# pepborrell/cool-chic

Measured on AMD Instinct MI355X. Metric: decoded Mpixel/s (Synth+ARM+upsample) @1280x720, all GPUs, higher is better.
Workload: dtype f32; 1 GPU; 1280x720 YUV420 8-bit frames, hop/c3x decoder (arm 16x2, syn 48-1/3-1/3-3r/3-3r, 7 latent grids), float forward ARM+rate -> upsampling -> synthesis -> 420 post; parallelism=image-parallel x1, kernels=ARM | upsampling pyramid | fused last-upsampling+synthesis+post (one stream)

## Files before the change

### cool-chic_amd/ccmi/__init__.py

```python

from __future__ import annotations

import ctypes as C
import os
from pathlib import Path

PKG_ROOT = Path(__file__).resolve().parents[1]
LIB_PATH = Path(os.environ.get("CCMI_LIB", PKG_ROOT / "lib" / "libccmi.so"))

MAX_GRIDS = 8
MAX_SYN_LAYERS = 16

OK, ERR_ARG, ERR_HIP, ERR_UNSUPPORTED, ERR_BITSTREAM, ERR_IO = range(6)

EXPORTED = [
    "ccmi_last_error", "ccmi_version", "ccmi_device_count",
    "ccmi_arm_forward_f32", "ccmi_arm_context_f32", "ccmi_arm_mlp_f32", "ccmi_ups_workspace_bytes", "ccmi_ups_forward_f32",
    "ccmi_syn_workspace_bytes", "ccmi_syn_forward_f32", "ccmi_post_f32", "ccmi_decode_forward_f32",
    "ccmi_fused_run_plan",
    "ccmi_decode_file", "ccmi_decode_batch", "ccmi_decode_output_size", "ccmi_decode_last_timing",
    "ccmi_decode_last_arm_flags", "ccmi_decode_latents", "ccmi_decode_batch_workspace_bytes", "ccmi_decode_batch_plan", "ccmi_decode_batch_ws", "ccmi_decode_weights_i32",
    "ccmi_decode_batch_dev_plan", "ccmi_decode_batch_dev", "ccmi_decode_batch_dev_roi_plan", "ccmi_decode_batch_dev_roi",
    "ccmi_latents_plan", "ccmi_latents_decode", "ccmi_latents_free", "ccmi_latents_count", "ccmi_latents_values",
    "ccmi_latents_render_plan", "ccmi_latents_render",
    "ccmi_latents_compact_plan", "ccmi_latents_compact_measure", "ccmi_latents_compact", "ccmi_latents_concat",
    "ccmi_latents_stream_info",
    "ccmi_latents_file_head", "ccmi_latents_export_plan", "ccmi_latents_export", "ccmi_latents_import_plan",
    "ccmi_latents_import",
    "ccmi_decode_batch_dev_fmt_plan", "ccmi_decode_batch_dev_fmt", "ccmi_latents_render_fmt_plan", "ccmi_latents_render_fmt",
    "ccmi_decode_batch_dev_rs_plan", "ccmi_decode_batch_dev_rs", "ccmi_latents_render_rs_plan", "ccmi_latents_render_rs",
    "ccmi_decode_last_tail_groups",
    "ccmi_decode_batch_dev_warp_plan", "ccmi_decode_batch_dev_warp", "ccmi_latents_render_warp_plan", "ccmi_latents_render_warp",
    "ccmi_decode_batch_dev_col_plan", "ccmi_decode_batch_dev_col", "ccmi_latents_render_col_plan", "ccmi_latents_render_col",
    "ccmi_ups_workspace_bytes_i32", "ccmi_ups_forward_i32", "ccmi_syn_workspace_bytes_i32", "ccmi_syn_forward_i32",
    "ccmi_cool_parse", "ccmi_code_wb", "ccmi_decode_wb", "ccmi_code_latent_layer", "ccmi_arm_forward_i32",
    "ccmi_encode_frame", "ccmi_row_reduce_f32", "ccmi_train_param_count", "ccmi_train_workspace_bytes", "ccmi_train_step",
    "ccmi_quantize_f32",
]


class CcmiUnavailable(RuntimeError):
    pass


class CcmiError(RuntimeError):
    def __init__(self, code: int, msg: str):
        super().__init__(f"ccmi error {code}: {msg}")
        self.code = code


class ArmArgs(C.Structure):
    _fields_ = [
        ("latent", C.c_void_p), ("latent_stride", C.c_int64), ("n_grids", C.c_int),
        ("h", C.c_int * MAX_GRIDS), ("w", C.c_int * MAX_GRIDS), ("gain", C.c_float),
        ("quantize", C.c_int), ("dim_arm", C.c_int), ("n_hidden", C.c_int),
        ("params", C.c_void_p), ("param_stride", C.c_int64),
        ("mu", C.c_void_p), ("scale", C.c_void_p), ("log_scale", C.c_void_p), ("rate", C.c_void_p),
        ("out_stride", C.c_int64), ("batch", C.c_int),
    ]


class UpsArgs(C.Structure):
    _fields_ = [
        ("latent", C.c_void_p), ("latent_stride", C.c_int64), ("n_grids", C.c_int),
        ("h", C.c_int * MAX_GRIDS), ("w", C.c_int * MAX_GRIDS), ("gain", C.c_float),
        ("quantize", C.c_int), ("ups_k", C.c_int), ("n_ups", C.c_int), ("pre_k", C.c_int),
        ("n_pre", C.c_int), ("params", C.c_void_p), ("param_stride", C.c_int64),
        ("out", C.c_void_p), ("out_stride", C.c_int64), ("workspace", C.c_void_p),
        ("workspace_bytes", C.c_size_t), ("batch", C.c_int),
    ]


class SynLayer(C.Structure):
    _fields_ = [("n_out", C.c_int), ("ks", C.c_int), ("residual", C.c_int), ("relu", C.c_int)]


class SynArgs(C.Structure):
    _fields_ = [
        ("in_", C.c_void_p), ("in_stride", C.c_int64), ("c_in", C.c_int), ("h", C.c_int), ("w", C.c_int),
        ("n_layers", C.c_int), ("layers", SynLayer * MAX_SYN_LAYERS), ("params", C.c_void_p),
        ("param_stride", C.c_int64), ("out", C.c_void_p), ("out_stride", C.c_int64),
        ("workspace", C.c_void_p), ("workspace_bytes", C.c_size_t), ("batch", C.c_int),
    ]


class PostArgs(C.Structure):
    _fields_ = [
        ("in_", C.c_void_p), ("in_stride", C.c_int64), ("h", C.c_int), ("w", C.c_int),
        ("bitdepth", C.c_int), ("yuv420", C.c_int), ("out", C.c_void_p), ("out_stride", C.c_int64),
        ("batch", C.c_int),
    ]


class DecodeArgs(C.Structure):
    _fields_ = [
        ("ups", UpsArgs), ("syn", SynArgs), ("bitdepth", C.c_int), ("yuv420", C.c_int),
        ("out", C.c_void_p), ("out_stride", C.c_int64), ("stages", C.c_int), ("head", C.c_int),
    ]


HEAD_DEFAULT, HEAD_VALU, HEAD_MFMA, HEAD_GENERIC = 0, 1, 2, 3


_lib = None


def lib() -> C.CDLL:
    global _lib
    if _lib is not None:
        return _lib
    try:
        import torch
    except ImportError:
        pass
    if not LIB_PATH.exists():
        raise CcmiUnavailable(f"{LIB_PATH} not built: run `make -C cool-chic_amd` (or __graft_entry__.build())")
    L = C.CDLL(str(LIB_PATH))
    L.ccmi_last_error.restype = C.c_char_p
    L.ccmi_version.restype = C.c_int
    L.ccmi_device_count.restype = C.c_int
    for name, st in (("ccmi_arm_forward_f32", ArmArgs), ("ccmi_ups_forward_f32", UpsArgs),
                     ("ccmi_syn_forward_f32", SynArgs), ("ccmi_post_f32", PostArgs),
                     ("ccmi_decode_forward_f32", DecodeArgs)):
        f = getattr(L, name)
        f.argtypes = [C.POINTER(st), C.c_void_p]
        f.restype = C.c_int
    L.ccmi_arm_context_f32.argtypes = [C.c_void_p, C.c_int, C.c_int, C.c_int, C.c_int, C.c_void_p, C.c_void_p]
    L.ccmi_arm_context_f32.restype = C.c_int
    L.ccmi_arm_mlp_f32.argtypes = [C.c_void_p, C.c_int64, C.c_int, C.c_int, C.c_void_p, C.c_void_p, C.c_void_p,
                                   C.c_void_p, C.c_void_p]
    L.ccmi_arm_mlp_f32.restype = C.c_int
    L.ccmi_ups_workspace_bytes.argtypes = [C.c_int, C.POINTER(C.c_int), C.POINTER(C.c_int), C.c_int]
    L.ccmi_ups_workspace_bytes.restype = C.c_size_t
    L.ccmi_syn_workspace_bytes.argtypes = [C.POINTER(SynArgs)]
    L.ccmi_syn_workspace_bytes.restype = C.c_size_t
    L.ccmi_decode_file.argtypes = [C.c_char_p, C.c_char_p, C.c_int, C.c_int, C.c_int, C.c_int]
    L.ccmi_decode_file.restype = C.c_int
    L.ccmi_decode_batch.argtypes = [C.POINTER(C.c_void_p), C.POINTER(C.c_size_t), C.c_int,
                                    C.POINTER(C.c_void_p), C.POINTER(C.c_size_t), C.POINTER(C.c_size_t),
                                    C.c_int, C.c_int, C.c_int, C.c_void_p]
    L.ccmi_decode_batch.restype = C.c_int
    L.ccmi_decode_output_size.argtypes = [C.c_void_p, C.c_size_t, C.c_int, C.c_int, C.c_int,
                                          C.POINTER(C.c_size_t)]
    L.ccmi_decode_output_size.restype = C.c_int
    L.ccmi_decode_last_timing.argtypes = [C.POINTER(C.c_float)]
    L.ccmi_decode_last_timing.restype = C.c_int
    if hasattr(L, "ccmi_fused_run_plan"):
        L.ccmi_fused_run_plan.argtypes = [C.c_int, C.c_int, C.c_int, C.POINTER(C.c_int), C.POINTER(C.c_int), C.c_int,
                                          C.POINTER(C.c_int)]
        L.ccmi_fused_run_plan.restype = C.c_int
    if hasattr(L, "ccmi_decode_last_arm_flags"):
        L.ccmi_decode_last_arm_flags.argtypes = [C.POINTER(C.c_uint32), C.c_int, C.POINTER(C.c_int)]
        L.ccmi_decode_last_arm_flags.restype = C.c_int
    _lib = L
    return L


def check(rc: int) -> None:
    if rc != OK:
        raise CcmiError(rc, lib().ccmi_last_error().decode(errors="replace"))


def last_error() -> str:
    return lib().ccmi_last_error().decode(errors="replace")


def __getattr__(name):
    if name == "LatentStore":
        from .decode import LatentStore
        return LatentStore
    raise AttributeError(f"module 'ccmi' has no attribute {name!r}")


def stream_handle(device=None) -> int:
    import torch
    return torch.cuda.current_stream(device).cuda_stream


def ptr(t) -> int:
# ... 12 lines not shown
```

### cool-chic_amd/ccmi/forward.py

```python

from __future__ import annotations

import ctypes
from typing import Sequence

import torch

from . import (ArmArgs, DecodeArgs, MAX_GRIDS, MAX_SYN_LAYERS, PostArgs, SynArgs, SynLayer, UpsArgs, check, lib, ptr,
               require_cuda, stream_handle)


def _grid_arrays(sizes: Sequence[tuple[int, int]]):
    if not 1 <= len(sizes) <= MAX_GRIDS:
        raise ValueError(f"1..{MAX_GRIDS} latent grids supported, got {len(sizes)}")
    h = (ctypes.c_int * MAX_GRIDS)()
    w = (ctypes.c_int * MAX_GRIDS)()
    for i, (hh, ww) in enumerate(sizes):
        h[i], w[i] = int(hh), int(ww)
    return h, w


def n_latents(sizes) -> int:
    return sum(int(h) * int(w) for h, w in sizes)


def arm_param_count(dim_arm: int, n_hidden: int) -> int:
    return n_hidden * (dim_arm * dim_arm + dim_arm) + 2 * dim_arm + 2


def pack_arm(layers: Sequence[tuple[torch.Tensor, torch.Tensor]]) -> torch.Tensor:
    return torch.cat([t.reshape(-1).float() for wb in layers for t in wb])


def pack_ups(ups: Sequence[torch.Tensor], pre: Sequence[torch.Tensor]) -> torch.Tensor:
    return torch.cat([k.reshape(-1).float() for k in list(ups) + list(pre)])


def pack_syn(layers: Sequence[tuple[torch.Tensor, torch.Tensor]]) -> torch.Tensor:
    return torch.cat([t.reshape(-1).float() for wb in layers for t in wb])


def _as_batch(params: torch.Tensor, B: int):
    if params.dim() == 1:
        return params.unsqueeze(0), 0
    if params.shape[0] != B:
        raise ValueError(f"params: expected {B} parameter rows, got {params.shape[0]}")
    return params, params.shape[1]


def arm_forward(latent: torch.Tensor, sizes, params: torch.Tensor, dim_arm: int, n_hidden: int,
                gain: float = 16.0, quantize: bool = True, want=("mu", "scale", "log_scale", "rate")) -> dict:
    squeeze = latent.dim() == 1
    latent = latent.unsqueeze(0) if squeeze else latent
    B, N = latent.shape
    params, pstride = _as_batch(params, B)
    require_cuda(latent, params)
    if N != n_latents(sizes):
        raise ValueError(f"latent has {N} values, grids hold {n_latents(sizes)}")
    if params.shape[1] < arm_param_count(dim_arm, n_hidden):
        raise ValueError("arm params: expected [B, >=%d]" % arm_param_count(dim_arm, n_hidden))
    latent = latent.float().contiguous()
    params = params.float().contiguous()
    outs = {k: torch.empty(B, N, device=latent.device, dtype=torch.float32) for k in want}
    h, w = _grid_arrays(sizes)
    a = ArmArgs(latent=ptr(latent), latent_stride=N, n_grids=len(sizes), h=h, w=w, gain=float(gain),
                quantize=int(bool(quantize)), dim_arm=dim_arm, n_hidden=n_hidden, params=ptr(params),
                param_stride=pstride, mu=ptr(outs.get("mu")), scale=ptr(outs.get("scale")),
                log_scale=ptr(outs.get("log_scale")), rate=ptr(outs.get("rate")), out_stride=N, batch=B)
    check(lib().ccmi_arm_forward_f32(a, stream_handle(latent.device)))
    if squeeze:
        outs = {k: v[0] for k, v in outs.items()}
    return outs


def ups_forward(latent: torch.Tensor, sizes, params: torch.Tensor, ups_k: int, n_ups: int, pre_k: int, n_pre: int,
                gain: float = 16.0, quantize: bool = True) -> torch.Tensor:
    squeeze = latent.dim() == 1
    latent = latent.unsqueeze(0) if squeeze else latent
    B, N = latent.shape
    params, pstride = _as_batch(params, B)
    require_cuda(latent, params)
    if N != n_latents(sizes):
        raise ValueError(f"latent has {N} values, grids hold {n_latents(sizes)}")
    if params.shape[1] < n_ups * ups_k + n_pre * pre_k:
        raise ValueError("ups params: wrong shape")
    latent = latent.float().contiguous()
    params = params.float().contiguous()
    L = len(sizes)
    H, W = sizes[0]
    out = torch.empty(B, L, H, W, device=latent.device, dtype=torch.float32)
    h, w = _grid_arrays(sizes)
    nws = lib().ccmi_ups_workspace_bytes(L, h, w, B)
    ws = torch.empty(max(nws, 4), device=latent.device, dtype=torch.uint8)
    a = UpsArgs(latent=ptr(latent), latent_stride=N, n_grids=L, h=h, w=w, gain=float(gain),
                quantize=int(bool(quantize)), ups_k=ups_k, n_ups=n_ups, pre_k=pre_k, n_pre=n_pre,
                params=ptr(params), param_stride=pstride, out=ptr(out), out_stride=L * H * W,
                workspace=ptr(ws), workspace_bytes=nws, batch=B)
    check(lib().ccmi_ups_forward_f32(a, stream_handle(latent.device)))
    return out[0] if squeeze else out


def _syn_args(x, layers, params, out, B, C, H, W, pstride=None):
    if len(layers) > MAX_SYN_LAYERS:
        raise ValueError("too many synthesis layers")
    arr = (SynLayer * MAX_SYN_LAYERS)()
    for i, (n_out, ks, res, relu) in enumerate(layers):
        arr[i] = SynLayer(int(n_out), int(ks), int(bool(res)), int(bool(relu)))
    return SynArgs(in_=ptr(x), in_stride=C * H * W, c_in=C, h=H, w=W, n_layers=len(layers), layers=arr,
                   params=ptr(params), param_stride=params.shape[1] if pstride is None else pstride, out=ptr(out),
                   out_stride=out.shape[1] * H * W, workspace=None, workspace_bytes=0, batch=B)


def syn_param_count(c_in: int, layers) -> int:
    n, c = 0, c_in
    for n_out, ks, _, _ in layers:
        n += n_out * c * ks * ks + n_out
        c = n_out
    return n


def syn_forward(x: torch.Tensor, layers, params: torch.Tensor) -> torch.Tensor:
    squeeze = x.dim() == 3
# ... 124 lines not shown
```

### cool-chic_amd/csrc/ccmi_api.cpp

```cpp
#include <stdarg.h>
#include <stdio.h>

#include <mutex>

#include "ccmi_internal.h"

static thread_local char g_err[512] = "";

int ccmi_set_error(int code, const char *fmt, ...)
{
    va_list ap;
    va_start(ap, fmt);
    vsnprintf(g_err, sizeof g_err, fmt, ap);
    va_end(ap);
    return code;
}

static std::mutex g_pool_mu;
static std::vector<StreamSet *> g_pool;

StreamSet *ccmi_streamset_acquire(int nst, int nev, bool timing)
{
    int dev = 0;
    if (hipGetDevice(&dev) != hipSuccess) {
        ccmi_set_error(CCMI_ERR_HIP, "stream pool: hipGetDevice failed");
        return nullptr;
    }
    {
        std::lock_guard<std::mutex> lk(g_pool_mu);
        for (size_t i = 0; i < g_pool.size(); ++i) {
            StreamSet *s = g_pool[i];
            if (s->device == dev && s->timing == timing && (int)s->st.size() >= nst && (int)s->ev.size() >= nev) {
                g_pool.erase(g_pool.begin() + (long)i);
                return s;
            }
        }
    }
    StreamSet *s = new StreamSet;
    s->device = dev;
    s->timing = timing;
    s->st.assign(nst, nullptr);
    s->ev.assign(nev, nullptr);
    bool ok = true;
    for (auto &x : s->st) ok = ok && hipStreamCreateWithFlags(&x, hipStreamNonBlocking) == hipSuccess;
    for (auto &x : s->ev) ok = ok && (timing ? hipEventCreate(&x) : hipEventCreateWithFlags(&x, hipEventDisableTiming)) == hipSuccess;
    if (!ok) {
        ccmi_set_error(CCMI_ERR_HIP, "stream pool: stream / event creation failed");
        for (auto x : s->st)
            if (x) (void)hipStreamDestroy(x);
        for (auto x : s->ev)
            if (x) (void)hipEventDestroy(x);
        delete s;
        return nullptr;
    }
    return s;
}

void ccmi_streamset_release(StreamSet *set)
{
    std::lock_guard<std::mutex> lk(g_pool_mu);
    g_pool.push_back(set);
}

extern "C" const char *ccmi_last_error(void) { return g_err; }

extern "C" int ccmi_version(void) { return 101; }

extern "C" int ccmi_device_count(void)
{
    int n = 0;
    if (hipGetDeviceCount(&n) != hipSuccess) return 0;
    return n;
}

static int check_grids(int n, const int *h, const int *w, const char *who)
{
    if (n < 1 || n > CCMI_MAX_GRIDS) return ccmi_set_error(CCMI_ERR_ARG, "%s: n_grids must be in [1, %d]", who, CCMI_MAX_GRIDS);
    for (int l = 0; l < n; ++l)
        if (h[l] < 1 || w[l] < 1) return ccmi_set_error(CCMI_ERR_ARG, "%s: grid %d has size %dx%d", who, l, h[l], w[l]);
    return CCMI_OK;
}

extern "C" int ccmi_arm_forward_f32(const ccmi_arm_args *a, void *stream)
{
    if (!a || !a->latent || !a->params) return ccmi_set_error(CCMI_ERR_ARG, "arm: null argument");
    if (int rc = check_grids(a->n_grids, a->h, a->w, "arm")) return rc;
    if (a->batch < 1) return ccmi_set_error(CCMI_ERR_ARG, "arm: batch must be >= 1");
    if (a->n_hidden < 0 || a->n_hidden > 4) return ccmi_set_error(CCMI_ERR_UNSUPPORTED, "arm: n_hidden must be in [0, 4]");
    const int64_t need = (int64_t)a->n_hidden * (a->dim_arm * a->dim_arm + a->dim_arm) + 2 * a->dim_arm + 2;
    if (a->param_stride != 0 && a->param_stride < need) return ccmi_set_error(CCMI_ERR_ARG, "arm: param_stride < %lld", (long long)need);
    if (!a->rate && !a->mu && !a->scale && !a->log_scale) return ccmi_set_error(CCMI_ERR_ARG, "arm: no output requested");
    return ccmi_launch_arm_f32(a, static_cast<hipStream_t>(stream));
}

extern "C" int ccmi_ups_forward_f32(const ccmi_ups_args *a, void *stream)
{
    if (!a || !a->latent || !a->params || !a->out) return ccmi_set_error(CCMI_ERR_ARG, "ups: null argument");
    if (int rc = check_grids(a->n_grids, a->h, a->w, "ups")) return rc;
    if (a->batch < 1) return ccmi_set_error(CCMI_ERR_ARG, "ups: batch must be >= 1");
    return ccmi_launch_ups_f32(a, static_cast<hipStream_t>(stream));
}

extern "C" int ccmi_syn_forward_f32(const ccmi_syn_args *a, void *stream)
{
    if (!a || !a->in || !a->params || !a->out) return ccmi_set_error(CCMI_ERR_ARG, "syn: null argument");
    if (a->h < 1 || a->w < 1 || a->c_in < 1 || a->batch < 1) return ccmi_set_error(CCMI_ERR_ARG, "syn: bad shape");
    return ccmi_launch_syn_f32(a, static_cast<hipStream_t>(stream));
}

extern "C" int ccmi_post_f32(const ccmi_post_args *a, void *stream)
{
    if (!a || !a->in || !a->out) return ccmi_set_error(CCMI_ERR_ARG, "post: null argument");
    if (a->h < 1 || a->w < 1 || a->batch < 1) return ccmi_set_error(CCMI_ERR_ARG, "post: bad shape");
    return ccmi_launch_post_f32(a, static_cast<hipStream_t>(stream));
}
```

### cool-chic_amd/csrc/ccmi_internal.h

```cpp
#pragma once

#include <hip/hip_runtime.h>
#include <stdint.h>

#include <vector>

#include "../../include/ccmi.h"

#define CCMI_MAX_GRIDS 8

struct GridGeom {
    int n;
    int h[CCMI_MAX_GRIDS];
    int w[CCMI_MAX_GRIDS];
    int off[CCMI_MAX_GRIDS];
    int total;
};

int ccmi_set_error(int code, const char *fmt, ...);

#define CCMI_HIP_CHECK(expr)                                                                \
    do {                                                                                    \
        hipError_t _e = (expr);                                                             \
        if (_e != hipSuccess)                                                               \
            return ccmi_set_error(CCMI_ERR_HIP, "%s failed: %s", #expr, hipGetErrorString(_e)); \
    } while (0)

static inline int ccmi_div_up(int a, int b) { return (a + b - 1) / b; }

int ccmi_launch_arm_f32(const ccmi_arm_args *a, hipStream_t s);
int ccmi_launch_ups_f32(const ccmi_ups_args *a, hipStream_t s);
int ccmi_launch_syn_f32(const ccmi_syn_args *a, hipStream_t s);
int ccmi_launch_post_f32(const ccmi_post_args *a, hipStream_t s);

struct StreamSet {
    int device = -1;
    bool timing = false;
    std::vector<hipStream_t> st;
    std::vector<hipEvent_t> ev;
};
StreamSet *ccmi_streamset_acquire(int nst, int nev, bool timing);
void ccmi_streamset_release(StreamSet *set);
struct StreamSetLease {
    StreamSet *set = nullptr;
    StreamSetLease() = default;
    StreamSetLease(const StreamSetLease &) = delete;
    StreamSetLease &operator=(const StreamSetLease &) = delete;
    ~StreamSetLease()
    {
        if (set) ccmi_streamset_release(set);
    }
};
```

### cool-chic_amd/csrc/fwd_arm.hip

```cpp
#include <stdlib.h>

#include <algorithm>

#include "fwd_common.h"

using ccmi_fwd::cfloat_ptr;
using ccmi_fwd::f2;

namespace {

constexpr int kThreads = 256;
constexpr int kTX = 64;
constexpr int kRowsPerPass = kThreads / kTX;
#ifndef CCMI_ARM_NL
#define CCMI_ARM_NL 2
#endif
constexpr int kNL = CCMI_ARM_NL;
constexpr int kNP = kNL / 2;
constexpr int kTY = kRowsPerPass * kNL;
constexpr int kHalo = 4;
constexpr int kLW = kTX + 2 * kHalo;
constexpr int kLH = kTY + kHalo;


struct ArmGeom {
    int n;
    int h[CCMI_MAX_GRIDS], w[CCMI_MAX_GRIDS], off[CCMI_MAX_GRIDS];
    int tiles_x[CCMI_MAX_GRIDS];
    int tile_start[CCMI_MAX_GRIDS + 1];
};

template <int D>
__device__ __forceinline__ void ctx_offset(int i, int &dy, int &dx)
{
    constexpr signed char k8[8] = {13, 22, 30, 31, 32, 37, 38, 39};
    constexpr signed char k16[16] = {13, 14, 20, 21, 22, 23, 24, 28, 29, 30, 31, 32, 33, 37, 38, 39};
    constexpr signed char k24[24] = {4, 11, 12, 13, 14, 15, 19, 20, 21, 22, 23, 24, 25, 28, 29, 30, 31, 32, 33, 34,
                                     36, 37, 38, 39};
    constexpr signed char k32[32] = {2, 3, 4, 5, 10, 11, 12, 13, 14, 15, 16, 19, 20, 21, 22, 23, 24, 25, 26, 27,
                                     28, 29, 30, 31, 32, 33, 34, 35, 36, 37, 38, 39};
    int k = D == 8 ? k8[i] : D == 16 ? k16[i] : D == 24 ? k24[i] : k32[i];
    dy = k / 9 - 4;
    dx = k % 9 - 4;
}

__device__ __forceinline__ float laplace_cdf(float x, float mu, float inv_scale)
{
    float s = x - mu;
    float sg = s > 0.f ? 1.f : (s < 0.f ? -1.f : 0.f);
    return 0.5f - 0.5f * sg * (__expf(-fabsf(s) * inv_scale) - 1.f);
}

template <int D, int NH = -1>
__global__ __launch_bounds__(kThreads) void arm_fwd_kernel(
    const float *__restrict__ lat, int64_t lat_stride, ArmGeom g, float gain, int quantize, int nh,
    const float *__restrict__ params, int64_t pstride, float *__restrict__ o_mu, float *__restrict__ o_scale,
    float *__restrict__ o_log_scale, float *__restrict__ o_rate, int64_t ostride)
{
    __shared__ float tile[kLH][kLW];

    const int wt = ccmi_fwd::xcd_order(blockIdx.x, gridDim.x);
    const int ntl = g.tile_start[g.n];
    const int b = wt / ntl;
    const int t = wt - b * ntl;
    int l = 0;
#pragma unroll
    for (int k = 1; k < CCMI_MAX_GRIDS; ++k)
        if (k < g.n && t >= g.tile_start[k]) l = k;
    const int lt = t - g.tile_start[l];
    const int H = g.h[l], W = g.w[l];
    const int y0 = (lt / g.tiles_x[l]) * kTY;
    const int x0 = (lt % g.tiles_x[l]) * kTX;
    const float *src = lat + (int64_t)b * lat_stride + g.off[l];

    {
        constexpr int NU = (kLH * kLW + kThreads - 1) / kThreads;
        float lv[NU];
#pragma unroll
        for (int u = 0; u < NU; ++u) {
            const int i = threadIdx.x + u * kThreads;
            const int r = i / kLW, c = i - r * kLW;
            const int y = y0 - kHalo + r, x = x0 - kHalo + c;
            lv[u] = (i < kLH * kLW && y >= 0 && y < H && x >= 0 && x < W) ? src[y * W + x] : 0.f;
        }
#pragma unroll
        for (int u = 0; u < NU; ++u) {
            const int i = threadIdx.x + u * kThreads;
            if (i < kLH * kLW) tile[i / kLW][i % kLW] = quantize ? rintf(gain * lv[u]) : lv[u];
        }
    }
    __syncthreads();

    const cfloat_ptr p = (cfloat_ptr)(size_t)(params + (int64_t)b * pstride);
    const int cx = threadIdx.x % kTX;
    const int cy0 = threadIdx.x / kTX;

    static_assert(kNL % 2 == 0, "packed pair layout");
    f2 a[kNP][D];
#pragma unroll
    for (int i = 0; i < D; ++i) {
        int dy, dx;
        ctx_offset<D>(i, dy, dx);
#pragma unroll
        for (int q = 0; q < kNP; ++q)
            a[q][i] = f2{tile[cy0 + 2 * q * kRowsPerPass + kHalo + dy][cx + kHalo + dx],
                         tile[cy0 + (2 * q + 1) * kRowsPerPass + kHalo + dy][cx + kHalo + dx]};
    }

    if constexpr (NH >= 0) nh = NH;
#pragma unroll
    for (int layer = 0; layer < nh; ++layer) {
        const cfloat_ptr Wl = p + layer * (D * D + D);
        const cfloat_ptr bl = Wl + D * D;
        f2 o[kNP][D];
#pragma unroll
        for (int j = 0; j < D; ++j) {
            f2 acc[kNP];
#pragma unroll
            for (int q = 0; q < kNP; ++q) acc[q] = a[q][j] + f2(bl[j]);
#pragma unroll
            for (int i = 0; i < D; ++i) {
                const f2 wji = f2(Wl[j * D + i]);
#pragma unroll
                for (int q = 0; q < kNP; ++q) acc[q] = __builtin_elementwise_fma(wji, a[q][i], acc[q]);
            }
#pragma unroll
            for (int q = 0; q < kNP; ++q) o[q][j] = __builtin_elementwise_max(acc[q], f2(0.f));
        }
#pragma unroll
        for (int q = 0; q < kNP; ++q)
#pragma unroll
            for (int j = 0; j < D; ++j) a[q][j] = o[q][j];
    }

    const cfloat_ptr Wo = p + nh * (D * D + D);
    f2 m[kNP], ls[kNP];
#pragma unroll
    for (int q = 0; q < kNP; ++q) {
        m[q] = f2(Wo[2 * D]);
        ls[q] = f2(Wo[2 * D + 1]);
    }
#pragma unroll
    for (int i = 0; i < D; ++i) {
        const f2 w0 = f2(Wo[i]), w1 = f2(Wo[D + i]);
#pragma unroll
        for (int q = 0; q < kNP; ++q) {
            m[q] = __builtin_elementwise_fma(w0, a[q][i], m[q]);
            ls[q] = __builtin_elementwise_fma(w1, a[q][i], ls[q]);
        }
    }
#pragma unroll
    for (int n = 0; n < kNL; ++n) {
        const int y = y0 + cy0 + n * kRowsPerPass, x = x0 + cx;
        const float mn = (n & 1) ? m[n >> 1].y : m[n >> 1].x, lsn = (n & 1) ? ls[n >> 1].y : ls[n >> 1].x;
        if (y < H && x < W) {
            const float sc = __expf(fminf(fmaxf(lsn - 4.f, -4.6f), 5.0f));
            const float q = tile[cy0 + n * kRowsPerPass + kHalo][cx + kHalo];
            const int64_t idx = (int64_t)b * ostride + g.off[l] + y * W + x;
            if (o_mu) o_mu[idx] = mn;
            if (o_scale) o_scale[idx] = sc;
            if (o_log_scale) o_log_scale[idx] = lsn;
            if (o_rate) {
                const float is = __builtin_amdgcn_rcpf(sc);
                const float pr = fmaxf(laplace_cdf(q + 0.5f, mn, is) - laplace_cdf(q - 0.5f, mn, is), 1.52587890625e-05f);
                o_rate[idx] = -__log2f(pr);
            }
        }
    }
}

template <int D>
__global__ __launch_bounds__(kThreads) void arm_context_kernel(const float *__restrict__ grid, int H, int W,
                                                               float *__restrict__ out)
{
    const int b = blockIdx.y;
    const int64_t p = (int64_t)blockIdx.x * kThreads + threadIdx.x;
    if (p >= (int64_t)H * W) return;
    const int y = (int)(p / W), x = (int)(p - (int64_t)y * W);
    const float *g = grid + (int64_t)b * H * W;
    float *o = out + ((int64_t)b * H * W + p) * D;
#pragma unroll
    for (int i = 0; i < D; ++i) {
        int dy, dx;
        ctx_offset<D>(i, dy, dx);
        const int yy = y + dy, xx = x + dx;
        o[i] = (yy >= 0 && xx >= 0 && xx < W) ? g[yy * W + xx] : 0.f;
    }
}

template <int D>
__global__ __launch_bounds__(kThreads) void arm_mlp_kernel(const float *__restrict__ ctx, int64_t M, int nh,
                                                           const float *__restrict__ p, float *__restrict__ o_mu,
                                                           float *__restrict__ o_scale, float *__restrict__ o_ls)
{
    const int64_t r = (int64_t)blockIdx.x * kThreads + threadIdx.x;
    if (r >= M) return;
    float a[D];
#pragma unroll
    for (int i = 0; i < D; ++i) a[i] = ctx[r * D + i];
    for (int layer = 0; layer < nh; ++layer) {
        const float *Wl = p + layer * (D * D + D);
        float o[D];
#pragma unroll
        for (int j = 0; j < D; ++j) {
            float acc = 0.f;
#pragma unroll
            for (int i = 0; i < D; ++i) acc = fmaf(Wl[j * D + i], a[i], acc);
            o[j] = fmaxf((acc + Wl[D * D + j]) + a[j], 0.f);
        }
#pragma unroll
        for (int j = 0; j < D; ++j) a[j] = o[j];
    }
    const float *Wo = p + nh * (D * D + D);
    float m = 0.f, ls = 0.f;
#pragma unroll
    for (int i = 0; i < D; ++i) {
        m = fmaf(Wo[i], a[i], m);
        ls = fmaf(Wo[D + i], a[i], ls);
    }
    m += Wo[2 * D];
    ls += Wo[2 * D + 1];
    if (o_mu) o_mu[r] = m;
    if (o_ls) o_ls[r] = ls;
    if (o_scale) o_scale[r] = expf(fminf(fmaxf(ls - 4.f, -4.6f), 5.0f));
}

}

extern "C" int ccmi_arm_context_f32(const float *grid, int batch, int h, int w, int dim_arm, float *out, void *stream)
{
    if (!grid || !out || batch < 1 || h < 1 || w < 1) return ccmi_set_error(CCMI_ERR_ARG, "arm_context: bad argument");
    dim3 g((unsigned)(((int64_t)h * w + kThreads - 1) / kThreads), batch);
    hipStream_t s = static_cast<hipStream_t>(stream);
    switch (dim_arm) {
    case 8: hipLaunchKernelGGL(arm_context_kernel<8>, g, dim3(kThreads), 0, s, grid, h, w, out); break;
    case 16: hipLaunchKernelGGL(arm_context_kernel<16>, g, dim3(kThreads), 0, s, grid, h, w, out); break;
    case 24: hipLaunchKernelGGL(arm_context_kernel<24>, g, dim3(kThreads), 0, s, grid, h, w, out); break;
    case 32: hipLaunchKernelGGL(arm_context_kernel<32>, g, dim3(kThreads), 0, s, grid, h, w, out); break;
    default: return ccmi_set_error(CCMI_ERR_UNSUPPORTED, "arm_context: dim_arm %d", dim_arm);
    }
    CCMI_HIP_CHECK(hipGetLastError());
    return CCMI_OK;
}

extern "C" int ccmi_arm_mlp_f32(const float *ctx, int64_t m, int dim_arm, int n_hidden, const float *params, float *mu,
                                float *scale, float *log_scale, void *stream)
{
    if (!ctx || !params || m < 0 || n_hidden < 0 || n_hidden > 4) return ccmi_set_error(CCMI_ERR_ARG, "arm_mlp: bad argument");
    if (m == 0) return CCMI_OK;
    dim3 g((unsigned)((m + kThreads - 1) / kThreads));
    hipStream_t s = static_cast<hipStream_t>(stream);
    switch (dim_arm) {
    case 8: hipLaunchKernelGGL(arm_mlp_kernel<8>, g, dim3(kThreads), 0, s, ctx, m, n_hidden, params, mu, scale, log_scale); break;
    case 16: hipLaunchKernelGGL(arm_mlp_kernel<16>, g, dim3(kThreads), 0, s, ctx, m, n_hidden, params, mu, scale, log_scale); break;
    case 24: hipLaunchKernelGGL(arm_mlp_kernel<24>, g, dim3(kThreads), 0, s, ctx, m, n_hidden, params, mu, scale, log_scale); break;
    case 32: hipLaunchKernelGGL(arm_mlp_kernel<32>, g, dim3(kThreads), 0, s, ctx, m, n_hidden, params, mu, scale, log_scale); break;
    default: return ccmi_set_error(CCMI_ERR_UNSUPPORTED, "arm_mlp: dim_arm %d", dim_arm);
    }
    CCMI_HIP_CHECK(hipGetLastError());
    return CCMI_OK;
}

int ccmi_launch_arm_f32(const ccmi_arm_args *a, hipStream_t s)
{
    ArmGeom g{};
    g.n = a->n_grids;
    int off = 0, tiles = 0;
    for (int l = 0; l < a->n_grids; ++l) {
        g.h[l] = a->h[l];
        g.w[l] = a->w[l];
        g.off[l] = off;
        g.tiles_x[l] = ccmi_div_up(a->w[l], kTX);
        g.tile_start[l] = tiles;
        tiles += g.tiles_x[l] * ccmi_div_up(a->h[l], kTY);
        off += a->h[l] * a->w[l];
    }
    g.tile_start[a->n_grids] = tiles;
    if ((a->latent_stride != 0 && a->latent_stride < off) || a->out_stride < off)
        return ccmi_set_error(CCMI_ERR_ARG, "arm: stride smaller than the %d latents of a frame", off);
    dim3 grid((unsigned)(tiles * a->batch));
#define CCMI_ARM_LAUNCH(DD)                                                                                     \
    hipLaunchKernelGGL(arm_fwd_kernel<DD>, grid, dim3(kThreads), 0, s, a->latent, a->latent_stride, g, a->gain, \
                       a->quantize, a->n_hidden, a->params, a->param_stride, a->mu, a->scale, a->log_scale,     \
                       a->rate, a->out_stride)
    switch (a->dim_arm) {
    case 8: CCMI_ARM_LAUNCH(8); break;
    case 16:
        if (a->n_hidden == 2) {
            hipLaunchKernelGGL((arm_fwd_kernel<16, 2>), grid, dim3(kThreads), 0, s, a->latent, a->latent_stride, g, a->gain,
                               a->quantize, a->n_hidden, a->params, a->param_stride, a->mu, a->scale, a->log_scale,
                               a->rate, a->out_stride);
        } else {
            CCMI_ARM_LAUNCH(16);
        }
        break;
    case 24: CCMI_ARM_LAUNCH(24); break;
    case 32: CCMI_ARM_LAUNCH(32); break;
    default: return ccmi_set_error(CCMI_ERR_UNSUPPORTED, "arm: dim_arm must be 8, 16, 24 or 32 (got %d)", a->dim_arm);
    }
#undef CCMI_ARM_LAUNCH
    CCMI_HIP_CHECK(hipGetLastError());
    return CCMI_OK;
}
```

### cool-chic_amd/csrc/fwd_common.h

```cpp
#pragma once

#include "ccmi_internal.h"

namespace ccmi_fwd {

typedef float f2 __attribute__((ext_vector_type(2)));
typedef const __attribute__((address_space(4))) float *cfloat_ptr;

__device__ __forceinline__ int clampi(int v, int hi) { return v < 0 ? 0 : (v > hi ? hi : v); }

__device__ __forceinline__ int xcd_order(int i, int n)
{
    const int per = (n + 7) >> 3, rem = n & 7, xcd = i & 7;
    return (rem == 0 ? xcd * per : xcd * per - max(0, xcd - rem)) + (i >> 3);
}

constexpr int kMaxIn = 8;
constexpr int kMaxMid = 4;
constexpr int kMaxSp = 3;
constexpr int kMaxHid = 64;

struct SpLayer {
    int w_off, b_off;
    int residual, relu;
};

struct FusedArgs {
    const float *in;
    int64_t in_stride;
    int cin, H, W;
    int n_head;
    int hid;
    int head_mfma;
    int head_generic;
    int ntiles;
    int run_base, run_extra;
    int w0_off, b0_off, relu0;
    int w1_off, b1_off, relu1;
    int n_sp;
    SpLayer sp[kMaxSp];
    const float *params;
    int64_t pstride;
    float *out;
    int64_t out_stride;
    int tiles_x;
    float qmax;
    int yuv420;
};

struct Plan {
    bool fused;
    int hid, cmid;
    FusedArgs fa;
};

#ifndef CCMI_FUSED_RUN
#define CCMI_FUSED_RUN 6
#endif
struct RunPlan {
    int n_runs, base, extra;
};
inline RunPlan fused_run_plan(int H, int h, int R, int rh)
{
    if (h == 0 || R < 1) R = 1;
    const int per = rh * R - 2 * h;
    const int n_runs = (H + per - 1) / per;
    const int windows = (H + 2 * h * n_runs + rh - 1) / rh;
// ... 46 lines not shown
```

### include/ccmi.h

```cpp
#ifndef CCMI_H
#define CCMI_H

#include <stddef.h>
#include <stdint.h>

#ifdef __cplusplus
extern "C" {
#endif

#define CCMI_OK 0
#define CCMI_ERR_ARG 1
#define CCMI_ERR_HIP 2
#define CCMI_ERR_UNSUPPORTED 3
#define CCMI_ERR_BITSTREAM 4
#define CCMI_ERR_IO 5

#define CCMI_MAX_GRIDS_PUBLIC 8
#define CCMI_MAX_SYN_LAYERS 16

const char *ccmi_last_error(void);
int ccmi_version(void);
int ccmi_device_count(void);


typedef struct ccmi_arm_args {
    const float *latent;
    int64_t latent_stride;
    int n_grids;
    int h[CCMI_MAX_GRIDS_PUBLIC];
    int w[CCMI_MAX_GRIDS_PUBLIC];
    float gain;
    int quantize;
    int dim_arm;
    int n_hidden;
    const float *params;
    int64_t param_stride;
    float *mu;
    float *scale;
    float *log_scale;
    float *rate;
    int64_t out_stride;
    int batch;
} ccmi_arm_args;
int ccmi_arm_forward_f32(const ccmi_arm_args *args, void *stream);

int ccmi_arm_context_f32(const float *grid, int batch, int h, int w, int dim_arm, float *out, void *stream);
int ccmi_arm_mlp_f32(const float *ctx, int64_t m, int dim_arm, int n_hidden, const float *params, float *mu,
                     float *scale, float *log_scale, void *stream);

typedef struct ccmi_ups_args {
    const float *latent;
    int64_t latent_stride;
    int n_grids;
    int h[CCMI_MAX_GRIDS_PUBLIC];
    int w[CCMI_MAX_GRIDS_PUBLIC];
    float gain;
    int quantize;
    int ups_k;
    int n_ups;
    int pre_k;
    int n_pre;
    const float *params;
    int64_t param_stride;
    float *out;
    int64_t out_stride;
    void *workspace;
    size_t workspace_bytes;
    int batch;
} ccmi_ups_args;
size_t ccmi_ups_workspace_bytes(int n_grids, const int *h, const int *w, int batch);
int ccmi_ups_forward_f32(const ccmi_ups_args *args, void *stream);

typedef struct ccmi_syn_layer {
    int n_out;
    int ks;
    int residual;
    int relu;
} ccmi_syn_layer;

typedef struct ccmi_syn_args {
    const float *in;
    int64_t in_stride;
    int c_in;
    int h;
    int w;
    int n_layers;
    ccmi_syn_layer layers[CCMI_MAX_SYN_LAYERS];
    const float *params;
    int64_t param_stride;
    float *out;
    int64_t out_stride;
    void *workspace;
    size_t workspace_bytes;
    int batch;
} ccmi_syn_args;
size_t ccmi_syn_workspace_bytes(const ccmi_syn_args *args);
int ccmi_syn_forward_f32(const ccmi_syn_args *args, void *stream);
// ... 369 lines not shown
```

Measured before the change: 24460 Mpixel/s.

## Add packed-weight pairs form for ARM MLP with scaled quantized arithmetic

Adds a new ARM forward kernel that first repacks the MLP weights into padded, transposed rows in a per-stream device buffer. Each thread then streams those weights through scalar registers with software prefetch and packed FMA over two latents. When quantizing, values are prescaled by 2^-32 so the ReLU can fold into a clamp on the last FMA. This path becomes the default for dim_arm 8 or 16, replacing the per-row kernel and aiming to cut VALU and weight-load cost in the ARM stage. In exchange it adds an extra pack kernel launch per call and relies on the scaled-clamp trick matching ReLU numerically.

```diff
diff --git a/cool-chic_amd/ccmi/__init__.py b/cool-chic_amd/ccmi/__init__.py
--- a/cool-chic_amd/ccmi/__init__.py
+++ b/cool-chic_amd/ccmi/__init__.py
@@ -15,7 +15,7 @@
 
 EXPORTED = [
     "ccmi_last_error", "ccmi_version", "ccmi_device_count",
-    "ccmi_arm_forward_f32", "ccmi_arm_context_f32", "ccmi_arm_mlp_f32", "ccmi_ups_workspace_bytes", "ccmi_ups_forward_f32",
+    "ccmi_arm_forward_f32", "ccmi_arm_forward_f32_form", "ccmi_arm_pack_host", "ccmi_arm_context_f32", "ccmi_arm_mlp_f32", "ccmi_ups_workspace_bytes", "ccmi_ups_forward_f32",
     "ccmi_syn_workspace_bytes", "ccmi_syn_forward_f32", "ccmi_post_f32", "ccmi_decode_forward_f32",
     "ccmi_fused_run_plan",
     "ccmi_decode_file", "ccmi_decode_batch", "ccmi_decode_output_size", "ccmi_decode_last_timing",
@@ -99,6 +99,7 @@
     ]
 
 
+ARM_FORM_DEFAULT, ARM_FORM_ROWS, ARM_FORM_PAIRS = 0, 1, 2
 HEAD_DEFAULT, HEAD_VALU, HEAD_MFMA, HEAD_GENERIC = 0, 1, 2, 3
 
 
@@ -125,6 +126,11 @@
         f = getattr(L, name)
         f.argtypes = [C.POINTER(st), C.c_void_p]
         f.restype = C.c_int
+    if hasattr(L, "ccmi_arm_forward_f32_form"):
+        L.ccmi_arm_forward_f32_form.argtypes = [C.POINTER(ArmArgs), C.c_void_p, C.c_int]
+        L.ccmi_arm_forward_f32_form.restype = C.c_int
+        L.ccmi_arm_pack_host.argtypes = [C.POINTER(C.c_float), C.c_int, C.c_int, C.POINTER(C.c_float)]
+        L.ccmi_arm_pack_host.restype = C.c_int
     L.ccmi_arm_context_f32.argtypes = [C.c_void_p, C.c_int, C.c_int, C.c_int, C.c_int, C.c_void_p, C.c_void_p]
     L.ccmi_arm_context_f32.restype = C.c_int
     L.ccmi_arm_mlp_f32.argtypes = [C.c_void_p, C.c_int64, C.c_int, C.c_int, C.c_void_p, C.c_void_p, C.c_void_p,
diff --git a/cool-chic_amd/ccmi/forward.py b/cool-chic_amd/ccmi/forward.py
--- a/cool-chic_amd/ccmi/forward.py
+++ b/cool-chic_amd/ccmi/forward.py
@@ -49,7 +49,8 @@
 
 
 def arm_forward(latent: torch.Tensor, sizes, params: torch.Tensor, dim_arm: int, n_hidden: int,
-                gain: float = 16.0, quantize: bool = True, want=("mu", "scale", "log_scale", "rate")) -> dict:
+                gain: float = 16.0, quantize: bool = True, want=("mu", "scale", "log_scale", "rate"),
+                form: int = 0) -> dict:
     squeeze = latent.dim() == 1
     latent = latent.unsqueeze(0) if squeeze else latent
     B, N = latent.shape
@@ -67,7 +68,10 @@
                 quantize=int(bool(quantize)), dim_arm=dim_arm, n_hidden=n_hidden, params=ptr(params),
                 param_stride=pstride, mu=ptr(outs.get("mu")), scale=ptr(outs.get("scale")),
                 log_scale=ptr(outs.get("log_scale")), rate=ptr(outs.get("rate")), out_stride=N, batch=B)
-    check(lib().ccmi_arm_forward_f32(a, stream_handle(latent.device)))
+    if form:
+        check(lib().ccmi_arm_forward_f32_form(a, stream_handle(latent.device), int(form)))
+    else:
+        check(lib().ccmi_arm_forward_f32(a, stream_handle(latent.device)))
     if squeeze:
         outs = {k: v[0] for k, v in outs.items()}
     return outs
diff --git a/cool-chic_amd/csrc/ccmi_api.cpp b/cool-chic_amd/csrc/ccmi_api.cpp
--- a/cool-chic_amd/csrc/ccmi_api.cpp
+++ b/cool-chic_amd/csrc/ccmi_api.cpp
@@ -62,6 +62,37 @@
     g_pool.push_back(set);
 }
 
+struct ArmPackBuf {
+    int device;
+    hipStream_t stream;
+    float *ptr;
+    size_t bytes;
+};
+static std::mutex g_pack_mu;
+static std::vector<ArmPackBuf> g_pack;
+
+int ccmi_arm_pack_buffer(size_t bytes, hipStream_t s, float **out)
+{
+    *out = nullptr;
+    int dev = 0;
+    CCMI_HIP_CHECK(hipGetDevice(&dev));
+    std::lock_guard<std::mutex> lk(g_pack_mu);
+    for (const ArmPackBuf &b : g_pack)
+        if (b.device == dev && b.stream == s && b.bytes >= bytes) {
+            *out = b.ptr;
+            return CCMI_OK;
+        }
+    hipStreamCaptureStatus cap = hipStreamCaptureStatusNone;
+    CCMI_HIP_CHECK(hipStreamIsCapturing(s, &cap));
+    if (cap != hipStreamCaptureStatusNone) return CCMI_OK;
+    const size_t want = (bytes + 65535) & ~(size_t)65535;
+    float *p = nullptr;
+    CCMI_HIP_CHECK(hipMalloc(reinterpret_cast<void **>(&p), want));
+    g_pack.insert(g_pack.begin(), ArmPackBuf{dev, s, p, want});
+    *out = p;
+    return CCMI_OK;
+}
+
 extern "C" const char *ccmi_last_error(void) { return g_err; }
 
 extern "C" int ccmi_version(void) { return 101; }
@@ -83,6 +114,12 @@
 
 extern "C" int ccmi_arm_forward_f32(const ccmi_arm_args *a, void *stream)
 {
+    return ccmi_arm_forward_f32_form(a, stream, CCMI_ARM_FORM_DEFAULT);
+}
+
+extern "C" int ccmi_arm_forward_f32_form(const ccmi_arm_args *a, void *stream, int form)
+{
+    if (form < CCMI_ARM_FORM_DEFAULT || form > CCMI_ARM_FORM_PAIRS) return ccmi_set_error(CCMI_ERR_ARG, "arm: unknown form %d", form);
     if (!a || !a->latent || !a->params) return ccmi_set_error(CCMI_ERR_ARG, "arm: null argument");
     if (int rc = check_grids(a->n_grids, a->h, a->w, "arm")) return rc;
     if (a->batch < 1) return ccmi_set_error(CCMI_ERR_ARG, "arm: batch must be >= 1");
@@ -90,7 +127,7 @@
     const int64_t need = (int64_t)a->n_hidden * (a->dim_arm * a->dim_arm + a->dim_arm) + 2 * a->dim_arm + 2;
     if (a->param_stride != 0 && a->param_stride < need) return ccmi_set_error(CCMI_ERR_ARG, "arm: param_stride < %lld", (long long)need);
     if (!a->rate && !a->mu && !a->scale && !a->log_scale) return ccmi_set_error(CCMI_ERR_ARG, "arm: no output requested");
-    return ccmi_launch_arm_f32(a, static_cast<hipStream_t>(stream));
+    return ccmi_launch_arm_f32(a, static_cast<hipStream_t>(stream), form);
 }
 
 extern "C" int ccmi_ups_forward_f32(const ccmi_ups_args *a, void *stream)
diff --git a/cool-chic_amd/csrc/ccmi_internal.h b/cool-chic_amd/csrc/ccmi_internal.h
--- a/cool-chic_amd/csrc/ccmi_internal.h
+++ b/cool-chic_amd/csrc/ccmi_internal.h
@@ -28,10 +28,12 @@
 
 static inline int ccmi_div_up(int a, int b) { return (a + b - 1) / b; }
 
-int ccmi_launch_arm_f32(const ccmi_arm_args *a, hipStream_t s);
+int ccmi_launch_arm_f32(const ccmi_arm_args *a, hipStream_t s, int form);
 int ccmi_launch_ups_f32(const ccmi_ups_args *a, hipStream_t s);
 int ccmi_launch_syn_f32(const ccmi_syn_args *a, hipStream_t s);
 int ccmi_launch_post_f32(const ccmi_post_args *a, hipStream_t s);
+
+int ccmi_arm_pack_buffer(size_t bytes, hipStream_t s, float **out);
 
 struct StreamSet {
     int device = -1;
diff --git a/cool-chic_amd/csrc/fwd_arm.hip b/cool-chic_amd/csrc/fwd_arm.hip
--- a/cool-chic_amd/csrc/fwd_arm.hip
+++ b/cool-chic_amd/csrc/fwd_arm.hip
@@ -23,6 +23,8 @@
 constexpr int kLH = kTY + kHalo;
 
 
+constexpr float kArmDown = 0x1p-32f, kArmUp = 0x1p+32f;
+
 struct ArmGeom {
     int n;
     int h[CCMI_MAX_GRIDS], w[CCMI_MAX_GRIDS], off[CCMI_MAX_GRIDS];
@@ -51,6 +53,75 @@
     return 0.5f - 0.5f * sg * (__expf(-fabsf(s) * inv_scale) - 1.f);
 }
 
+struct ArmTile {
+    int b, l, H, W, y0, x0;
+};
+
+template <bool SC = false>
+__device__ __forceinline__ ArmTile arm_stage_tile(float (&tile)[kLH][kLW], const float *__restrict__ lat,
+                                                  int64_t lat_stride, const ArmGeom &g, float gain, int quantize)
+{
+    const int wt = ccmi_fwd::xcd_order(blockIdx.x, gridDim.x);
+    const int ntl = g.tile_start[g.n];
+    ArmTile T;
+    T.b = wt / ntl;
+    const int t = wt - T.b * ntl;
+    int l = 0;
+#pragma unroll
+    for (int k = 1; k < CCMI_MAX_GRIDS; ++k)
+        if (k < g.n && t >= g.tile_start[k]) l = k;
+    const int lt = t - g.tile_start[l];
+    T.l = l;
+    T.H = g.h[l];
+    T.W = g.w[l];
+    T.y0 = (lt / g.tiles_x[l]) * kTY;
+    T.x0 = (lt % g.tiles_x[l]) * kTX;
+    const int H = T.H, W = T.W, y0 = T.y0, x0 = T.x0;
+    const float *src = lat + (int64_t)T.b * lat_stride + g.off[l];
+
+    {
+        constexpr int NU = (kLH * kLW + kThreads - 1) / kThreads;
+        float lv[NU];
+#pragma unroll
+        for (int u = 0; u < NU; ++u) {
+            const int i = threadIdx.x + u * kThreads;
+            const int r = i / kLW, c = i - r * kLW;
+            const int y = y0 - kHalo + r, x = x0 - kHalo + c;
+            lv[u] = (i < kLH * kLW && y >= 0 && y < H && x >= 0 && x < W) ? src[y * W + x] : 0.f;
+        }
+#pragma unroll
+        for (int u = 0; u < NU; ++u) {
+            const int i = threadIdx.x + u * kThreads;
+            if constexpr (SC) {
+                if (i < kLH * kLW) tile[i / kLW][i % kLW] = rintf(gain * lv[u]) * kArmDown;
+            } else {
+                if (i < kLH * kLW) tile[i / kLW][i % kLW] = quantize ? rintf(gain * lv[u]) : lv[u];
+            }
+        }
+    }
+    __syncthreads();
+    return T;
+}
+
+__device__ __forceinline__ void arm_emit(const ArmTile &T, const ArmGeom &g, int n, float mn, float lsn, float q,
+                                         float *__restrict__ o_mu, float *__restrict__ o_scale,
+                                         float *__restrict__ o_log_scale, float *__restrict__ o_rate, int64_t ostride)
+{
+    const int y = T.y0 + threadIdx.x / kTX + n * kRowsPerPass, x = T.x0 + threadIdx.x % kTX;
+    if (y < T.H && x < T.W) {
+        const float sc = __expf(fminf(fmaxf(lsn - 4.f, -4.6f), 5.0f));
+        const int64_t idx = (int64_t)T.b * ostride + g.off[T.l] + y * T.W + x;
+        if (o_mu) o_mu[idx] = mn;
+        if (o_scale) o_scale[idx] = sc;
+        if (o_log_scale) o_log_scale[idx] = lsn;
+        if (o_rate) {
+            const float is = __builtin_amdgcn_rcpf(sc);
+            const float pr = fmaxf(laplace_cdf(q + 0.5f, mn, is) - laplace_cdf(q - 0.5f, mn, is), 1.52587890625e-05f);
+            o_rate[idx] = -__log2f(pr);
+        }
+    }
+}
+
 template <int D, int NH = -1>
 __global__ __launch_bounds__(kThreads) void arm_fwd_kernel(
     const float *__restrict__ lat, int64_t lat_stride, ArmGeom g, float gain, int quantize, int nh,
@@ -58,40 +129,9 @@
     float *__restrict__ o_log_scale, float *__restrict__ o_rate, int64_t ostride)
 {
     __shared__ float tile[kLH][kLW];
-
-    const int wt = ccmi_fwd::xcd_order(blockIdx.x, gridDim.x);
-    const int ntl = g.tile_start[g.n];
-    const int b = wt / ntl;
-    const int t = wt - b * ntl;
-    int l = 0;
-#pragma unroll
-    for (int k = 1; k < CCMI_MAX_GRIDS; ++k)
-        if (k < g.n && t >= g.tile_start[k]) l = k;
-    const int lt = t - g.tile_start[l];
-    const int H = g.h[l], W = g.w[l];
-    const int y0 = (lt / g.tiles_x[l]) * kTY;
-    const int x0 = (lt % g.tiles_x[l]) * kTX;
-    const float *src = lat + (int64_t)b * lat_stride + g.off[l];
-
-    {
-        constexpr int NU = (kLH * kLW + kThreads - 1) / kThreads;
-        float lv[NU];
-#pragma unroll
-        for (int u = 0; u < NU; ++u) {
-            const int i = threadIdx.x + u * kThreads;
-            const int r = i / kLW, c = i - r * kLW;
-            const int y = y0 - kHalo + r, x = x0 - kHalo + c;
-            lv[u] = (i < kLH * kLW && y >= 0 && y < H && x >= 0 && x < W) ? src[y * W + x] : 0.f;
-        }
-#pragma unroll
-        for (int u = 0; u < NU; ++u) {
-            const int i = threadIdx.x + u * kThreads;
-            if (i < kLH * kLW) tile[i / kLW][i % kLW] = quantize ? rintf(gain * lv[u]) : lv[u];
-        }
-    }
-    __syncthreads();
-
-    const cfloat_ptr p = (cfloat_ptr)(size_t)(params + (int64_t)b * pstride);
+    const ArmTile T = arm_stage_tile(tile, lat, lat_stride, g, gain, quantize);
+
+    const cfloat_ptr p = (cfloat_ptr)(size_t)(params + (int64_t)T.b * pstride);
     const int cx = threadIdx.x % kTX;
     const int cy0 = threadIdx.x / kTX;
 
@@ -150,22 +190,146 @@
         }
     }
 #pragma unroll
+    for (int n = 0; n < kNL; ++n)
+        arm_emit(T, g, n, (n & 1) ? m[n >> 1].y : m[n >> 1].x, (n & 1) ? ls[n >> 1].y : ls[n >> 1].x,
+                 tile[cy0 + n * kRowsPerPass + kHalo][cx + kHalo], o_mu, o_scale, o_log_scale, o_rate, ostride);
+}
+
+__global__ __launch_bounds__(kThreads) void arm_pack_kernel(const float *__restrict__ params, int64_t pstride, int d,
+                                                            int nh, float *__restrict__ out, int ostride)
+{
+    const float *p = params + (int64_t)blockIdx.x * pstride;
+    float *o = out + (int64_t)blockIdx.x * ostride;
+    for (int t = threadIdx.x; t < ostride; t += kThreads) {
+        const int s = ccmi_fwd::arm_pack_src(d, nh, t);
+        o[t] = s >= 0 ? p[s] : 0.f;
+    }
+}
+
+template <int D>
+using arm_row = float __attribute__((ext_vector_type(D)));
+
+template <int D>
+__device__ __forceinline__ arm_row<D> arm_load_row(cfloat_ptr base, unsigned at, const arm_row<D> *landed = nullptr)
+{
+    if (landed) asm volatile("" ::"s"((*landed)[0]));
+    unsigned off = at * (unsigned)sizeof(float);
+    asm volatile("" : "+s"(off));
+    const arm_row<D> r =
+        *(const __attribute__((address_space(4))) arm_row<D> *)((const __attribute__((address_space(4))) char *)base + off);
+    __builtin_amdgcn_sched_barrier(0);
+    return r;
+}
+
+template <int N>
+__device__ __forceinline__ void arm_fence(f2 (&o)[kNL][N])
+{
+    static_assert(N == 4 || N == 8, "accumulator pairs per latent");
+#pragma unroll
     for (int n = 0; n < kNL; ++n) {
-        const int y = y0 + cy0 + n * kRowsPerPass, x = x0 + cx;
-        const float mn = (n & 1) ? m[n >> 1].y : m[n >> 1].x, lsn = (n & 1) ? ls[n >> 1].y : ls[n >> 1].x;
-        if (y < H && x < W) {
-            const float sc = __expf(fminf(fmaxf(lsn - 4.f, -4.6f), 5.0f));
-            const float q = tile[cy0 + n * kRowsPerPass + kHalo][cx + kHalo];
-            const int64_t idx = (int64_t)b * ostride + g.off[l] + y * W + x;
-            if (o_mu) o_mu[idx] = mn;
-            if (o_scale) o_scale[idx] = sc;
-            if (o_log_scale) o_log_scale[idx] = lsn;
-            if (o_rate) {
-                const float is = __builtin_amdgcn_rcpf(sc);
-                const float pr = fmaxf(laplace_cdf(q + 0.5f, mn, is) - laplace_cdf(q - 0.5f, mn, is), 1.52587890625e-05f);
-                o_rate[idx] = -__log2f(pr);
+        if constexpr (N == 8)
+            asm volatile("" : "+v"(o[n][0]), "+v"(o[n][1]), "+v"(o[n][2]), "+v"(o[n][3]), "+v"(o[n][4]), "+v"(o[n][5]),
+                         "+v"(o[n][6]), "+v"(o[n][7]));
+        else
+            asm volatile("" : "+v"(o[n][0]), "+v"(o[n][1]), "+v"(o[n][2]), "+v"(o[n][3]));
+    }
+}
+
+template <int D, int NH = -1, bool SC = false>
+__global__ __launch_bounds__(kThreads) void arm_fwd_pairs_kernel(
+    const float *__restrict__ lat, int64_t lat_stride, ArmGeom g, float gain, int quantize, int nh,
+    const float *__restrict__ packed, int pkstride, float *__restrict__ o_mu, float *__restrict__ o_scale,
+    float *__restrict__ o_log_scale, float *__restrict__ o_rate, int64_t ostride)
+{
+    static_assert(kNL == 2 && (D == 8 || D == 16), "pairs form: two latents per thread, dim_arm 8 or 16");
+    constexpr int RS = ccmi_fwd::arm_pack_row(D), LS = ccmi_fwd::arm_pack_layer(D), HP = D / 2;
+    __shared__ float tile[kLH][kLW];
+    const ArmTile T = arm_stage_tile<SC>(tile, lat, lat_stride, g, gain, quantize);
+
+    const cfloat_ptr P = (cfloat_ptr)(size_t)(packed + (int64_t)T.b * pkstride);
+    const int cx = threadIdx.x % kTX;
+    const int cy0 = threadIdx.x / kTX;
+    if constexpr (NH >= 0) nh = NH;
+
+    f2 a[kNL][HP];
+#pragma unroll
+    for (int i = 0; i < D; ++i) {
+        int dy, dx;
+        ctx_offset<D>(i, dy, dx);
+#pragma unroll
+        for (int n = 0; n < kNL; ++n) a[n][i >> 1][i & 1] = tile[cy0 + n * kRowsPerPass + kHalo + dy][cx + kHalo + dx];
+    }
+
+    const unsigned Wo = nh * LS;
+    const f2 bo = *(const __attribute__((address_space(4))) f2 *)(P + Wo + 2 * D);
+    arm_row<D> cur = arm_load_row<D>(P, nh > 0 ? D * RS : 0);
+#pragma unroll
+    for (int layer = 0; layer < nh; ++layer) {
+        const unsigned Wl = layer * LS;
+        f2 o[kNL][HP];
+        arm_row<D> nxt = arm_load_row<D>(P, Wl, &cur);
+#pragma unroll
+        for (int n = 0; n < kNL; ++n)
+#pragma unroll
+            for (int jp = 0; jp < HP; ++jp) {
+                const f2 bp = f2{cur[2 * jp], cur[2 * jp + 1]};
+                o[n][jp] = SC ? __builtin_elementwise_fma(bp, f2(kArmDown), a[n][jp]) : a[n][jp] + bp;
             }
-        }
+        arm_fence(o);
+        cur = nxt;
+#pragma unroll
+        for (int i = 0; i < D; ++i) {
+            nxt = arm_load_row<D>(P, i + 1 < D ? Wl + (i + 1) * RS : layer + 1 < nh ? Wl + LS + D * RS : Wl + LS, &cur);
+#pragma unroll
+            for (int n = 0; n < kNL; ++n) {
+                const f2 ai = f2(a[n][i >> 1][i & 1]);
+#pragma unroll
+                for (int jp = 0; jp < HP; ++jp) {
+                    const f2 wp = f2{cur[2 * jp], cur[2 * jp + 1]};
+                    if constexpr (SC && (D & 1) == 0) {
+                        if (i == D - 1) {
+                            asm("v_pk_fma_f32 %0, %1, %2, %3 op_sel:[0,1,0] op_sel_hi:[1,1,1] clamp"
+                                : "=v"(o[n][jp])
+                                : "s"(wp), "v"(a[n][HP - 1]), "v"(o[n][jp]));
+                            continue;
+                        }
+                    }
+                    o[n][jp] = __builtin_elementwise_fma(wp, ai, o[n][jp]);
+                }
+            }
+            if (i + 1 < D) arm_fence(o);
+            cur = nxt;
+        }
+#pragma unroll
+        for (int n = 0; n < kNL; ++n)
+#pragma unroll
+            for (int jp = 0; jp < HP; ++jp) a[n][jp] = SC ? o[n][jp] : __builtin_elementwise_max(o[n][jp], f2(0.f));
+    }
+
+    f2 ml[kNL];
+#pragma unroll
+    for (int n = 0; n < kNL; ++n) ml[n] = SC ? bo * kArmDown : bo;
+#pragma unroll
+    for (int half = 0; half < 2; ++half) {
+        arm_row<D> nxt = cur;
+        if (half == 0) nxt = arm_load_row<D>(P, Wo + D, &cur);
+#pragma unroll
+        for (int k = 0; k < HP; ++k) {
+            const int i = half * HP + k;
+#pragma unroll
+            for (int n = 0; n < kNL; ++n)
+                ml[n] = __builtin_elementwise_fma(f2{cur[2 * k], cur[2 * k + 1]}, f2(a[n][i >> 1][i & 1]), ml[n]);
+        }
+        cur = nxt;
+    }
+#pragma unroll
+    for (int n = 0; n < kNL; ++n) {
+        float q = tile[cy0 + n * kRowsPerPass + kHalo][cx + kHalo];
+        if constexpr (SC) {
+            ml[n] *= kArmUp;
+            q *= kArmUp;
+        }
+        arm_emit(T, g, n, ml[n].x, ml[n].y, q, o_mu, o_scale, o_log_scale, o_rate, ostride);
     }
 }
 
@@ -261,7 +425,18 @@
     return CCMI_OK;
 }
 
-int ccmi_launch_arm_f32(const ccmi_arm_args *a, hipStream_t s)
+extern "C" int ccmi_arm_pack_host(const float *params, int dim_arm, int n_hidden, float *out)
+{
+    if (!params || !out || dim_arm < 1 || n_hidden < 0) return -1;
+    const int n = ccmi_fwd::arm_pack_stride(dim_arm, n_hidden);
+    for (int t = 0; t < n; ++t) {
+        const int s = ccmi_fwd::arm_pack_src(dim_arm, n_hidden, t);
+        out[t] = s >= 0 ? params[s] : 0.f;
+    }
+    return n;
+}
+
+int ccmi_launch_arm_f32(const ccmi_arm_args *a, hipStream_t s, int form)
 {
     ArmGeom g{};
     g.n = a->n_grids;
@@ -279,6 +454,40 @@
     if ((a->latent_stride != 0 && a->latent_stride < off) || a->out_stride < off)
         return ccmi_set_error(CCMI_ERR_ARG, "arm: stride smaller than the %d latents of a frame", off);
     dim3 grid((unsigned)(tiles * a->batch));
+
+    const bool has_pairs = a->dim_arm == 8 || a->dim_arm == 16;
+    if (form == CCMI_ARM_FORM_PAIRS && !has_pairs)
+        return ccmi_set_error(CCMI_ERR_UNSUPPORTED, "arm: the pairs form needs dim_arm 8 or 16 (got %d)", a->dim_arm);
+    if (form != CCMI_ARM_FORM_ROWS && has_pairs) {
+        const int pks = ccmi_fwd::arm_pack_stride(a->dim_arm, a->n_hidden);
+        const int frames = a->param_stride ? a->batch : 1;
+        float *pk = nullptr;
+        if (int rc = ccmi_arm_pack_buffer((size_t)frames * pks * sizeof(float), s, &pk)) return rc;
+        if (!pk && form == CCMI_ARM_FORM_PAIRS)
+            return ccmi_set_error(CCMI_ERR_UNSUPPORTED, "arm: no packed-weight buffer for this stream while it captures");
+        if (pk) {
+            hipLaunchKernelGGL(arm_pack_kernel, dim3(frames), dim3(kThreads), 0, s, a->params, a->param_stride, a->dim_arm,
+                               a->n_hidden, pk, pks);
+#define CCMI_ARM_PAIRS(DD, NN)                                                                                        \
+    do {                                                                                                              \
+        auto kern = a->quantize ? arm_fwd_pairs_kernel<DD, NN, true> : arm_fwd_pairs_kernel<DD, NN, false>;          \
+        hipLaunchKernelGGL(kern, grid, dim3(kThreads), 0, s, a->latent, a->latent_stride, g, a->gain, a->quantize,   \
+                           a->n_hidden, pk, a->param_stride ? pks : 0, a->mu, a->scale, a->log_scale, a->rate,       \
+                           a->out_stride);                                                                           \
+    } while (0)
+            if (a->dim_arm == 8) {
+                if (a->n_hidden == 2) CCMI_ARM_PAIRS(8, 2);
+                else CCMI_ARM_PAIRS(8, -1);
+            } else {
+                if (a->n_hidden == 2) CCMI_ARM_PAIRS(16, 2);
+                else CCMI_ARM_PAIRS(16, -1);
+            }
+#undef CCMI_ARM_PAIRS
+            CCMI_HIP_CHECK(hipGetLastError());
+            return CCMI_OK;
+        }
+    }
+
 #define CCMI_ARM_LAUNCH(DD)                                                                                     \
     hipLaunchKernelGGL(arm_fwd_kernel<DD>, grid, dim3(kThreads), 0, s, a->latent, a->latent_stride, g, a->gain, \
                        a->quantize, a->n_hidden, a->params, a->param_stride, a->mu, a->scale, a->log_scale,     \
diff --git a/cool-chic_amd/csrc/fwd_common.h b/cool-chic_amd/csrc/fwd_common.h
--- a/cool-chic_amd/csrc/fwd_common.h
+++ b/cool-chic_amd/csrc/fwd_common.h
@@ -13,6 +13,22 @@
 {
     const int per = (n + 7) >> 3, rem = n & 7, xcd = i & 7;
     return (rem == 0 ? xcd * per : xcd * per - max(0, xcd - rem)) + (i >> 3);
+}
+
+constexpr int arm_pack_row(int d) { return (d + 15) & ~15; }
+constexpr int arm_pack_layer(int d) { return (d + 1) * arm_pack_row(d); }
+constexpr int arm_pack_stride(int d, int nh) { return (nh * arm_pack_layer(d) + 2 * d + 2 + 15) & ~15; }
+__host__ __device__ constexpr int arm_pack_src(int d, int nh, int t)
+{
+    const int rs = arm_pack_row(d), ls = arm_pack_layer(d), lp = d * d + d;
+    if (t < nh * ls) {
+        const int l = t / ls, r = t - l * ls, i = r / rs, j = r - i * rs;
+        if (j >= d) return -1;
+        return l * lp + (i < d ? j * d + i : d * d + j);
+    }
+    const int u = t - nh * ls;
+    if (u < 2 * d) return nh * lp + (u & 1) * d + (u >> 1);
+    return u < 2 * d + 2 ? nh * lp + u : -1;
 }
 
 constexpr int kMaxIn = 8;
diff --git a/include/ccmi.h b/include/ccmi.h
--- a/include/ccmi.h
+++ b/include/ccmi.h
@@ -43,6 +43,12 @@
     int batch;
 } ccmi_arm_args;
 int ccmi_arm_forward_f32(const ccmi_arm_args *args, void *stream);
+
+#define CCMI_ARM_FORM_DEFAULT 0
+#define CCMI_ARM_FORM_ROWS 1
+#define CCMI_ARM_FORM_PAIRS 2
+int ccmi_arm_forward_f32_form(const ccmi_arm_args *args, void *stream, int form);
+int ccmi_arm_pack_host(const float *params, int dim_arm, int n_hidden, float *out);
 
 int ccmi_arm_context_f32(const float *grid, int batch, int h, int w, int dim_arm, float *out, void *stream);
 int ccmi_arm_mlp_f32(const float *ctx, int64_t m, int dim_arm, int n_hidden, const float *params, float *mu,
```

Result: faster. 25270 Mpixel/s, median of 6 (+3.3%).
